# ChuyueL/advanced-hpc-lbm

Hardware: NVIDIA B200
Metric: MLUPS (d2q9-bgk lattice updates per second / 1e6) (higher is better)
Workload: dtype f32

## Files before the change

### advanced-hpc-lbm_b200/csrc/lbm_gpu.cu

```cuda
#include "lbm_gpu.h"
#include "lbm_kernels.cuh"
#include "lbm_cluster.cuh"
#include "lbm_tb2.cuh"
#include "lbm_tb3.cuh"
#include "lbm_pairs.cuh"
#include "lbm_f16.cuh"

#include <unistd.h>

#include <algorithm>
#include <cmath>
#include <cstdarg>
#include <cstdio>
#include <cstdlib>
#include <cstring>
#include <exception>
#include <memory>
#include <mutex>
#include <numeric>
#include <string>
#include <vector>

namespace {

thread_local std::string g_error;

struct CachedWindow { int device; size_t bytes; char* ptr; };
std::mutex g_window_mutex;
std::vector<CachedWindow> g_window_cache;
struct CachedIpcMapping { cudaIpcMemHandle_t handle; int device; void* ptr; };
std::vector<CachedIpcMapping> g_ipc_cache;

int fail(const char* fmt, ...) {
  char buf[1024];
  va_list ap;
  va_start(ap, fmt);
  vsnprintf(buf, sizeof buf, fmt, ap);
  va_end(ap);
  g_error = buf;
  return 1;
}

struct CudaError {
  std::string what;
};

#define CK(call)                                                                              \
  do {                                                                                        \
    cudaError_t e_ = (call);                                                                  \
    if (e_ != cudaSuccess) {                                                                  \
      char b_[512];                                                                           \
      snprintf(b_, sizeof b_, "CUDA error %s (%s) at %s:%d: %s", cudaGetErrorName(e_),        \
               cudaGetErrorString(e_), __FILE__, __LINE__, #call);                            \
      throw CudaError{b_};                                                                    \
    }                                                                                         \
  } while (0)

inline long long round_up(long long v, long long m) { return (v + m - 1) / m * m; }

inline bool env_on(const char* name) { const char* e = getenv(name); return e && e[0] == '1'; }

unsigned forced_kernel(unsigned flags) {
  static const char* const names[] = {nullptr, nullptr, "SCALAR", "TMA", "VEC4", nullptr, "PERSISTENT", nullptr, "CLUSTER", "TB2", nullptr, "PAIRS", "TB3"};
  unsigned k = 0;
  std::string msg = "more than one kernel forced, pass at most one of:";
  for (int b = 0; b < 13; b++)
    if (names[b] && (flags >> b & 1)) { k |= 1u << b; msg += std::string(" LBM_GPU_KERNEL_") + names[b]; }
  if (k & (k - 1)) throw CudaError{msg};
  return k;
}

constexpr int kPersistScalarBlocks = 296;
constexpr long long kPersistMaxCells = 1280 * 1024;
constexpr size_t kStagingBytes = 64u << 20;

struct IpcDesc {
  uint32_t magic;
  int32_t elem_size;
  int32_t device;
  int32_t pid;
  int32_t nx, pitch, rows;
  int32_t pad_;
  long long row0;
  unsigned long long win_addr;
  unsigned long long win_bytes;
  unsigned long long off_sync;
  unsigned long long off_gmask;
  unsigned long long steps_done;
  unsigned long long passes_done;
  long long local_free_cells;
  int32_t cur;
  int32_t tb2_ok;
  cudaIpcMemHandle_t handle;
  char gpu_uuid[16];
};
static_assert(sizeof(IpcDesc) <= LBM_GPU_IPC_DESC_BYTES, "descriptor too large");
constexpr uint32_t kIpcMagic = 0x4c424d31u;

enum SyncWord { kFlagFromBelow = 0, kFlagFromAbove = 1, kBoundaryDone = 2, kScratch0 = 3, kScratch1 = 4,
                kScratch2 = 5, kGridBarrier = 6, kAbort = 7, kSyncError = 8 ,
                kAvScratch = 16 , kSyncWords = 16 + 128 };
constexpr int kTb2MinRows = 8;
constexpr int kTb3MinRows = 12;
constexpr double kTb3MinWaves = 4.0;
constexpr int kAvWords = LBM_AV_STRIDE * LBM_AV_SLOTS;
constexpr int kMaxSegmentSteps = 1 << 16;

struct GridBase {
  virtual ~GridBase() {}
  virtual bool is_f64() const = 0;
};

template <typename real>
struct Slab {
  int device = 0;
  long long row0 = 0;
  int rows = 0;
  int accel_row = LBM_NO_ROW;
  char* base = nullptr;
  size_t bytes = 0;
  size_t off_lattice[2] = {0, 0}, off_side[2] = {0, 0}, off_mask = 0;
  real* lattice[2] = {nullptr, nullptr};
  real* side[2] = {nullptr, nullptr};
  uint32_t* mask = nullptr;
  char* win = nullptr;
  size_t win_bytes = 0, off_sync = 0, off_gmask = 0;
  unsigned long long* sync = nullptr;
  uint32_t* ghost_mask = nullptr;
  unsigned long long* av = nullptr;
  unsigned long long* av_compact = nullptr;
  size_t av_cap = 0;
  void* staging = nullptr;
  cudaStream_t stream = nullptr;
  cudaStream_t copy_stream = nullptr;
  cudaEvent_t stage_filled[2] = {nullptr, nullptr};
  cudaEvent_t stage_drained[2] = {nullptr, nullptr};
  cudaEvent_t ev0 = nullptr, ev1 = nullptr;
  cudaEvent_t step_ev[2] = {nullptr, nullptr};
  long long free_cells = 0;
  char* up_win = nullptr;
  char* dn_win = nullptr;
  unsigned long long* up_flag = nullptr;
  unsigned long long* dn_flag = nullptr;
  unsigned long long* up_abort = nullptr;
  unsigned long long* dn_abort = nullptr;
  uint32_t* up_gmask = nullptr;
  uint32_t* dn_gmask = nullptr;
  void* ipc_mapped[2] = {nullptr, nullptr};
  bool pooled = false;
  alignas(64) CUtensorMap tmap[2];
  alignas(64) CUtensorMap tmap_halo[2];
};

template <typename real> struct ParamT;
template <> struct ParamT<float> { typedef lbm_param type; };
template <> struct ParamT<double> { typedef lbm_param_f64 type; };

template <typename real>
class Grid : public GridBase {
 public:
  typedef typename ParamT<real>::type Param;
  Param prm;
  unsigned flags = 0;
  int kernel = 0;
  int persistent_vec = 4;
  int cluster_ctas = 0;
  int cluster_rows = 0;
  size_t cluster_smem = 0;
  int pitch = 0, mask_pitch = 0;
  bool slab_mode = false;
  bool connected = false;
  bool multi = false;
  bool use_flags = false;
  long long global_free_cells = -1;
  long long steps_done = 0;
  long long passes_done = 0;
  int cur = 0;
  int tb2_strips = 0, tb2_wout = 0, tb2_seg_rows = 0, tb2_span = 0, tb2_threads = 0;
  int tb2_tail_rows = 16, tb2_tail_segs = 0;
  int tb3_seg_rows = 0;
  int pairs_tile_rows = 0;
  bool f16 = false;
  bool failed = false;
  unsigned long long timeout_ns = 10000000000ULL;
  long long launches = 0;
  double last_run_ms = 0.0, last_step_ms = 0.0;
  std::vector<Slab<real>> slabs;

  bool is_f64() const override { return sizeof(real) == 8; }

  ~Grid() override {
    for (auto& s : slabs) {
      cudaSetDevice(s.device);
      if (s.stream) cudaStreamSynchronize(s.stream);
      for (int i = 0; i < 2; i++)
        if (s.ipc_mapped[i]) cudaIpcCloseMemHandle(s.ipc_mapped[i]);
      pool_free(s.av, s);
      pool_free(s.staging, s);
      pool_free(s.base, s);
      if (s.stream) cudaStreamSynchronize(s.stream);
      window_free(s);
      if (s.ev0) cudaEventDestroy(s.ev0);
      if (s.ev1) cudaEventDestroy(s.ev1);
      for (int i = 0; i < 2; i++) {
        if (s.stage_filled[i]) cudaEventDestroy(s.stage_filled[i]);
        if (s.stage_drained[i]) cudaEventDestroy(s.stage_drained[i]);
      }
      if (s.copy_stream) { cudaStreamSynchronize(s.copy_stream); cudaStreamDestroy(s.copy_stream); }
      for (int i = 0; i < 2; i++)
        if (s.step_ev[i]) cudaEventDestroy(s.step_ev[i]);
      if (s.stream) cudaStreamDestroy(s.stream);
    }
  }

  bool use_pool() const { return (flags & LBM_GPU_POOL) != 0; }
  void pool_alloc(void** p, size_t bytes, Slab<real>& s) {
    if (use_pool()) {
      int supported = 0;
      CK(cudaDeviceGetAttribute(&supported, cudaDevAttrMemoryPoolsSupported, s.device));
      if (supported) {
        cudaMemPool_t pool;
        CK(cudaDeviceGetDefaultMemPool(&pool, s.device));
        unsigned long long keep = ~0ULL;
        CK(cudaMemPoolSetAttribute(pool, cudaMemPoolAttrReleaseThreshold, &keep));
        CK(cudaMallocAsync(p, bytes, s.stream));
        s.pooled = true;
        return;
      }
    }
    CK(cudaMalloc(p, bytes));
  }
  static void pool_free(void* p, Slab<real>& s) {
    if (!p) return;
    if (s.pooled) cudaFreeAsync(p, s.stream);
    else cudaFree(p);
  }
  void window_alloc(Slab<real>& s) {
    if (use_pool()) {
      std::lock_guard<std::mutex> lock(g_window_mutex);
      for (size_t i = 0; i < g_window_cache.size(); i++)
        if (g_window_cache[i].device == s.device && g_window_cache[i].bytes == s.win_bytes) {
          s.win = g_window_cache[i].ptr;
          g_window_cache.erase(g_window_cache.begin() + i);
          return;
        }
    }
    CK(cudaMalloc((void**)&s.win, s.win_bytes));
  }
  void window_free(Slab<real>& s) {
    if (!s.win) return;
    if (use_pool()) {
      std::lock_guard<std::mutex> lock(g_window_mutex);
      g_window_cache.push_back({s.device, s.win_bytes, s.win});
    } else {
      cudaFree(s.win);
    }
    s.win = nullptr;
  }

  void alloc_slab(Slab<real>& s) {
    CK(cudaSetDevice(s.device));
    const long long plane = (long long)s.rows * pitch;
    const size_t lat = (size_t)9 * plane * (f16 ? sizeof(__half) : sizeof(real));
    const size_t side = (size_t)6 * pitch * sizeof(real);
    const size_t maskb = (size_t)s.rows * mask_pitch * sizeof(uint32_t);
    size_t off = 0;
    for (int i = 0; i < 2; i++) { s.off_lattice[i] = off; off = round_up(off + lat, 256); }
    for (int i = 0; i < 2; i++) { s.off_side[i] = off; off = round_up(off + side, 256); }
    s.off_mask = off; off = round_up(off + maskb, 256);
    s.bytes = off;
    CK(cudaStreamCreateWithFlags(&s.stream, cudaStreamNonBlocking));
    CK(cudaStreamCreateWithFlags(&s.copy_stream, cudaStreamNonBlocking));
    for (int i = 0; i < 2; i++) {
      CK(cudaEventCreateWithFlags(&s.stage_filled[i], cudaEventDisableTiming));
      CK(cudaEventCreateWithFlags(&s.stage_drained[i], cudaEventDisableTiming));
    }
    pool_alloc((void**)&s.base, s.bytes, s);
    for (int i = 0; i < 2; i++) {
      s.lattice[i] = (real*)(s.base + s.off_lattice[i]);
      s.side[i] = (real*)(s.base + s.off_side[i]);
    }
    s.mask = (uint32_t*)(s.base + s.off_mask);
    s.off_gmask = round_up((size_t)LBM_GHOST_PLANE_ROWS * pitch * sizeof(real), 256);
    s.off_sync = round_up(s.off_gmask + (size_t)2 * mask_pitch * sizeof(uint32_t), 256);
    s.win_bytes = round_up(s.off_sync + kSyncWords * sizeof(unsigned long long), 2u << 20);
    window_alloc(s);
    s.ghost_mask = (uint32_t*)(s.win + s.off_gmask);
    s.sync = (unsigned long long*)(s.win + s.off_sync);
    CK(cudaEventCreate(&s.ev0));
    CK(cudaEventCreate(&s.ev1));
    for (int i = 0; i < 2; i++) CK(cudaEventCreateWithFlags(&s.step_ev[i], cudaEventDisableTiming));
    CK(cudaMemsetAsync(s.base + s.off_side[0], 0, s.bytes - s.off_side[0], s.stream));
    CK(cudaMemsetAsync(s.win, 0, s.win_bytes, s.stream));
    void* st = nullptr;
    pool_alloc(&st, kStagingBytes, s);
    s.staging = st;
  }

  void make_tensor_maps(Slab<real>& s) {
    typedef CUresult (*EncodeFn)(CUtensorMap*, CUtensorMapDataType, cuuint32_t, void*, const cuuint64_t*,
                                 const cuuint64_t*, const cuuint32_t*, const cuuint32_t*, CUtensorMapInterleave,
                                 CUtensorMapSwizzle, CUtensorMapL2promotion, CUtensorMapFloatOOBfill);
    void* fn = nullptr;
    cudaDriverEntryPointQueryResult qres;
    CK(cudaGetDriverEntryPoint("cuTensorMapEncodeTiled", &fn, cudaEnableDefault, &qres));
    if (!fn || qres != cudaDriverEntryPointSuccess) throw CudaError{"cuTensorMapEncodeTiled is not available in this driver"};
    const cuuint64_t dims[3] = {(cuuint64_t)pitch, (cuuint64_t)s.rows, 9};
    const cuuint64_t strides[2] = {(cuuint64_t)pitch * sizeof(real), (cuuint64_t)plane_stride(s) * sizeof(real)};
    const cuuint32_t box[3] = {LBM_TMA_BOX, 1, 1};
    const cuuint32_t hbox[3] = {4, 1, 1};
    const cuuint32_t estr[3] = {1, 1, 1};
    for (int b = 0; b < 2; b++) {
      for (int h = 0; h < 2; h++) {
        const CUresult r = ((EncodeFn)fn)(h ? &s.tmap_halo[b] : &s.tmap[b], CU_TENSOR_MAP_DATA_TYPE_FLOAT32, 3, s.lattice[b],
                                          dims, strides, h ? hbox : box, estr, CU_TENSOR_MAP_INTERLEAVE_NONE,
                                          CU_TENSOR_MAP_SWIZZLE_NONE, CU_TENSOR_MAP_L2_PROMOTION_NONE,
                                          CU_TENSOR_MAP_FLOAT_OOB_FILL_NONE);
        if (r != CUDA_SUCCESS) {
          char msg[96];
          snprintf(msg, sizeof msg, "cuTensorMapEncodeTiled failed with CUresult %d", (int)r);
          throw CudaError{msg};
        }
      }
    }
  }

  real* win_section(char* win, int b, int d) const { return (real*)win + lbm::ghost_offset(pitch, b, d); }

  long long plane_stride(const Slab<real>& s) const { return (long long)s.rows * pitch; }

  __half* hlat(const Slab<real>& s, int b) const { return reinterpret_cast<__half*>(s.lattice[b]); }
  lbm::RestShift rest() const {
    lbm::RestShift r;
    r.w0 = (float)(prm.density * (real)4 / (real)9);
    r.w1 = (float)(prm.density / (real)9);
    r.w2 = (float)(prm.density / (real)36);
    return r;
  }

  void setup_geometry(int nx) {
    pitch = (int)round_up(nx, 32);
    mask_pitch = pitch / 32;
    if (const char* e = getenv("LBM_GPU_SYNC_TIMEOUT_MS")) {
      const double ms = atof(e);
      if (ms > 0) timeout_ns = (unsigned long long)(ms * 1e6);
    }
  }

  void tile_shape(int vec, int& bx, int& by) const {
    const int nxv = (prm.nx + vec - 1) / vec;
    bx = (int)std::min<long long>(LBM_BLOCK_THREADS, round_up(nxv, 32));
    if (kernel == LBM_GPU_KERNEL_TMA) bx = LBM_BLOCK_THREADS;
    by = LBM_BLOCK_THREADS / bx;
  }

  const void* persistent_fn() const {
    const bool strict = (flags & LBM_GPU_STRICT) != 0;
    if (persistent_vec == 1)
      return strict ? (const void*)lbm::lbm_steps_persistent<real, true, 1> : (const void*)lbm::lbm_steps_persistent<real, false, 1>;
    return strict ? (const void*)lbm::lbm_steps_persistent<real, true, 4> : (const void*)lbm::lbm_steps_persistent<real, false, 4>;
  }

  int persistent_capacity(const Slab<real>& s) {
    int per_sm = 0, sms = 0, coop = 0;
    CK(cudaOccupancyMaxActiveBlocksPerMultiprocessor(&per_sm, persistent_fn(), LBM_BLOCK_THREADS, 0));
    CK(cudaDeviceGetAttribute(&sms, cudaDevAttrMultiProcessorCount, s.device));
    CK(cudaDeviceGetAttribute(&coop, cudaDevAttrCooperativeLaunch, s.device));
    return coop ? per_sm * sms : 0;
  }

  const void* cluster_fn() const {
    return (flags & LBM_GPU_STRICT) ? (const void*)lbm::lbm_steps_cluster<true> : (const void*)lbm::lbm_steps_cluster<false>;
  }

  bool cluster_fits() {
    if (sizeof(real) != 4 || slabs.size() != 1 || slab_mode) return false;
    Slab<real>& s = slabs[0];
    int max_smem = 0;
    CK(cudaDeviceGetAttribute(&max_smem, cudaDevAttrMaxSharedMemoryPerBlockOptin, s.device));
    for (int c : {16, 8}) {
      const int rows = (s.rows + c - 1) / c;
      const size_t smem = (size_t)2 * 9 * rows * prm.nx * sizeof(float);
      if (smem > (size_t)max_smem) continue;
      if (cudaFuncSetAttribute(cluster_fn(), cudaFuncAttributeMaxDynamicSharedMemorySize, (int)smem) != cudaSuccess ||
          cudaFuncSetAttribute(cluster_fn(), cudaFuncAttributeNonPortableClusterSizeAllowed, 1) != cudaSuccess) {
        cudaGetLastError();
        continue;
      }
      cudaLaunchConfig_t cfg = {};
      cfg.gridDim = dim3(c);
      cfg.blockDim = dim3(LBM_CLUSTER_THREADS);
      cfg.dynamicSmemBytes = smem;
      cudaLaunchAttribute attr[1];
      attr[0].id = cudaLaunchAttributeClusterDimension;
      attr[0].val.clusterDim.x = c; attr[0].val.clusterDim.y = 1; attr[0].val.clusterDim.z = 1;
      cfg.attrs = attr;
      cfg.numAttrs = 1;
      int nclusters = 0;
      if (cudaOccupancyMaxActiveClusters(&nclusters, cluster_fn(), &cfg) != cudaSuccess || nclusters < 1) {
        cudaGetLastError();
        continue;
      }
      cluster_ctas = c;
      cluster_rows = rows;
      cluster_smem = smem;
      return true;
    }
// ... 1455 lines not shown
  return 0;
}

int lbm_gpu_ipc_export(lbm_gpu* h, void* desc) {
  if (!desc) return fail("lbm_gpu_ipc_export: NULL descriptor");
  return guarded<float>(h, "lbm_gpu_ipc_export", [&](Grid<float>& g) {
    if (g.slabs.size() != 1) throw CudaError{"only a one-slab handle can be exported"};
    if (g.f16) throw CudaError{"a LBM_GPU_STORE_F16 lattice cannot be shared between processes"};
    Slab<float>& s = g.slabs[0];
    CK(cudaSetDevice(s.device));
    IpcDesc d;
    memset(&d, 0, sizeof d);
    d.magic = kIpcMagic;
    d.elem_size = 4;
    d.device = s.device;
    d.pid = (int32_t)getpid();
    d.nx = g.prm.nx; d.pitch = g.pitch; d.rows = s.rows;
    d.row0 = s.row0;
    d.win_addr = (unsigned long long)(uintptr_t)s.win;
    d.win_bytes = s.win_bytes;
    d.off_sync = s.off_sync;
    d.off_gmask = s.off_gmask;
    d.steps_done = (unsigned long long)g.steps_done;
    d.passes_done = (unsigned long long)g.passes_done;
    d.local_free_cells = s.free_cells;
    d.cur = g.cur;
    d.tb2_ok = g.k7_fits(s.rows) ? 1 : 0;
    CK(cudaIpcGetMemHandle(&d.handle, s.win));
    cudaDeviceProp prop;
    CK(cudaGetDeviceProperties(&prop, s.device));
    memcpy(d.gpu_uuid, prop.uuid.bytes, 16);
    memset(desc, 0, LBM_GPU_IPC_DESC_BYTES);
    memcpy(desc, &d, sizeof d);
  });
}

namespace {
void ipc_connect_impl(Grid<float>& g, const IpcDesc& dn, const IpcDesc& up, bool ring_k7) {
  if (g.slabs.size() != 1) throw CudaError{"only a one-slab handle can be connected"};
  if (g.f16) throw CudaError{"a LBM_GPU_STORE_F16 lattice cannot be shared between processes"};
  Slab<float>& s = g.slabs[0];
  CK(cudaSetDevice(s.device));
  const long long ny = g.prm.ny;
  for (const IpcDesc* d : {&dn, &up}) {
    if (d->magic != kIpcMagic || d->elem_size != 4) throw CudaError{"bad neighbour descriptor"};
    if (d->nx != g.prm.nx || d->pitch != g.pitch) throw CudaError{"neighbour descriptor is for another grid width"};
    if (d->steps_done != (unsigned long long)g.steps_done || d->passes_done != (unsigned long long)g.passes_done ||
        d->cur != g.cur)
      throw CudaError{"neighbour is at a different timestep"};
  }
  cudaDeviceProp my_prop;
  CK(cudaGetDeviceProperties(&my_prop, s.device));
  for (const IpcDesc* d : {&dn, &up})
    if (memcmp(d->gpu_uuid, my_prop.uuid.bytes, 16) == 0 &&
        !(d->pid == (int32_t)getpid() && d->win_addr == (unsigned long long)(uintptr_t)s.win))
      throw CudaError{"a neighbouring slab runs on the same physical GPU: kernels that wait on one another "
                      "must not share a device (use lbm_gpu_create with n_gpus slabs in one process instead)"};
  if ((dn.row0 + dn.rows) % ny != s.row0 % ny) throw CudaError{"descriptor 'below' does not hold row0-1"};
  if ((s.row0 + s.rows) % ny != up.row0 % ny) throw CudaError{"descriptor 'above' does not hold row0+nrows"};
  auto map = [&](const IpcDesc& d, int slot) -> char* {
    if (d.pid == (int32_t)getpid()) {
      char* p = (char*)(uintptr_t)d.win_addr;
      if (p == s.win) return p;
      if (d.device == s.device)
        throw CudaError{"two slabs ordered by device-side flags must not share a GPU"};
      int can = 0;
      CK(cudaDeviceCanAccessPeer(&can, s.device, d.device));
      if (!can) throw CudaError{"peer access between the selected GPUs is not available"};
      cudaError_t e = cudaDeviceEnablePeerAccess(d.device, 0);
      if (e != cudaSuccess && e != cudaErrorPeerAccessAlreadyEnabled) CK(e);
      cudaGetLastError();
      return p;
    }
    if (g.use_pool()) {
      std::lock_guard<std::mutex> lock(g_window_mutex);
      for (auto& c : g_ipc_cache)
        if (c.device == s.device && memcmp(&c.handle, &d.handle, sizeof d.handle) == 0) return (char*)c.ptr;
    }
    void* p = nullptr;
    CK(cudaIpcOpenMemHandle(&p, d.handle, cudaIpcMemLazyEnablePeerAccess));
    if (g.use_pool()) {
      std::lock_guard<std::mutex> lock(g_window_mutex);
      g_ipc_cache.push_back({d.handle, s.device, p});
    } else {
      s.ipc_mapped[slot] = p;
    }
    return (char*)p;
  };
  for (const IpcDesc* d : {&dn, &up})
    if (d->win_bytes != s.win_bytes || d->off_sync != s.off_sync || d->off_gmask != s.off_gmask)
      throw CudaError{"neighbour window layout differs"};
  s.dn_win = map(dn, 0);
  s.up_win = (memcmp(&dn.handle, &up.handle, sizeof dn.handle) == 0 && dn.pid == up.pid) ? s.dn_win : map(up, 1);
  unsigned long long* dn_sync = (unsigned long long*)(s.dn_win + dn.off_sync);
  unsigned long long* up_sync = (unsigned long long*)(s.up_win + up.off_sync);
  s.dn_flag = dn_sync + kFlagFromAbove;
  s.up_flag = up_sync + kFlagFromBelow;
  s.dn_abort = dn_sync + kAbort;
  s.up_abort = up_sync + kAbort;
  s.dn_gmask = (uint32_t*)(s.dn_win + dn.off_gmask) + g.mask_pitch;
  s.up_gmask = (uint32_t*)(s.up_win + up.off_gmask);
  g.multi = true;
  g.use_flags = true;
  g.select_kernel(true, ring_k7);
  g.connected = true;
}
}

int lbm_gpu_ipc_connect(lbm_gpu* h, const void* desc_below, const void* desc_above) {
  if (!desc_below || !desc_above) return fail("lbm_gpu_ipc_connect: NULL descriptor");
  return guarded<float>(h, "lbm_gpu_ipc_connect", [&](Grid<float>& g) {
    IpcDesc dn, up;
    memcpy(&dn, desc_below, sizeof dn);
    memcpy(&up, desc_above, sizeof up);
    ipc_connect_impl(g, dn, up, false);
  });
}

int lbm_gpu_ipc_connect_all(lbm_gpu* h, const void* descs, int n) {
  if (!descs || n < 1) return fail("lbm_gpu_ipc_connect_all: bad argument");
  return guarded<float>(h, "lbm_gpu_ipc_connect_all", [&](Grid<float>& g) {
    if (g.slabs.size() != 1) throw CudaError{"only a one-slab handle can be connected"};
    Slab<float>& s = g.slabs[0];
    std::vector<IpcDesc> all(n);
    for (int i = 0; i < n; i++) memcpy(&all[i], (const char*)descs + (size_t)i * LBM_GPU_IPC_DESC_BYTES, sizeof(IpcDesc));
    const long long ny = g.prm.ny;
    long long rows_total = 0, free_total = 0;
    int below = -1, above = -1;
    bool all_k7 = true;
    for (int i = 0; i < n; i++) {
      const IpcDesc& d = all[i];
      if (d.magic != kIpcMagic) throw CudaError{"bad descriptor in the list"};
      rows_total += d.rows;
      free_total += d.local_free_cells;
      all_k7 = all_k7 && d.tb2_ok;
      if ((d.row0 + d.rows) % ny == s.row0 % ny) below = i;
      if ((s.row0 + s.rows) % ny == d.row0 % ny) above = i;
    }
    if (rows_total != ny) throw CudaError{"the descriptors do not cover the grid's rows exactly once"};
    if (below < 0 || above < 0) throw CudaError{"no descriptor holds the rows next to this slab"};
    ipc_connect_impl(g, all[below], all[above], all_k7);
    g.global_free_cells = free_total;
  });
}

int lbm_gpu_ipc_prepare(lbm_gpu* h) {
  return guarded<float>(h, "lbm_gpu_ipc_prepare", [&](Grid<float>& g) { g.prepare(); });
}

int lbm_gpu_run(lbm_gpu* h, int n_steps, float* av_vels_out) {
  return run_impl<float>(h, n_steps, av_vels_out, nullptr, "lbm_gpu_run");
}
int lbm_gpu_run_f64(lbm_gpu* h, int n_steps, double* av_vels_out) {
  return run_impl<double>(h, n_steps, av_vels_out, nullptr, "lbm_gpu_run_f64");
}
int lbm_gpu_run_batch(lbm_gpu* const* handles, int n, int n_steps, float* av_vels_out) {
  return run_batch_impl(handles, n, n_steps, av_vels_out);
}
int lbm_gpu_run_sums(lbm_gpu* h, int n_steps, double* sums_out) {
  if (!h) return fail("lbm_gpu_run_sums: NULL handle");
  if (reinterpret_cast<GridBase*>(h)->is_f64()) return run_impl<double>(h, n_steps, nullptr, sums_out, "lbm_gpu_run_sums");
  return run_impl<float>(h, n_steps, nullptr, sums_out, "lbm_gpu_run_sums");
}

int lbm_gpu_set_global_free_cells(lbm_gpu* h, long long free_cells) {
  if (!h) return fail("lbm_gpu_set_global_free_cells: NULL handle");
  if (free_cells < 1) return fail("lbm_gpu_set_global_free_cells: count must be positive");
  GridBase* b = reinterpret_cast<GridBase*>(h);
  if (b->is_f64()) static_cast<Grid<double>*>(b)->global_free_cells = free_cells;
  else static_cast<Grid<float>*>(b)->global_free_cells = free_cells;
  return 0;
}

int lbm_gpu_download(lbm_gpu* h, float* out) {
  if (!out) return fail("lbm_gpu_download: NULL output");
  return guarded<float>(h, "lbm_gpu_download", [&](Grid<float>& g) {
    long long rows = 0;
    for (auto& s : g.slabs) rows += s.rows;
    g.download_rows(g.slabs[0].row0, rows, out);
  });
}
int lbm_gpu_download_f64(lbm_gpu* h, double* out) {
  if (!out) return fail("lbm_gpu_download_f64: NULL output");
  return guarded<double>(h, "lbm_gpu_download_f64", [&](Grid<double>& g) {
    long long rows = 0;
    for (auto& s : g.slabs) rows += s.rows;
    g.download_rows(g.slabs[0].row0, rows, out);
  });
}
int lbm_gpu_download_rows(lbm_gpu* h, long long row0, long long nrows, float* out) {
  if (!out || nrows < 0) return fail("lbm_gpu_download_rows: bad argument");
  return guarded<float>(h, "lbm_gpu_download_rows", [&](Grid<float>& g) { g.download_rows(row0, nrows, out); });
}

int lbm_gpu_final_fields(lbm_gpu* h, long long row0, long long nrows, float* ux, float* uy, float* u, float* p) {
  if (nrows < 0) return fail("lbm_gpu_final_fields: bad argument");
  return guarded<float>(h, "lbm_gpu_final_fields", [&](Grid<float>& g) { g.final_fields(row0, nrows, ux, uy, u, p); });
}
int lbm_gpu_final_fields_f64(lbm_gpu* h, long long row0, long long nrows, double* ux, double* uy, double* u, double* p) {
  if (nrows < 0) return fail("lbm_gpu_final_fields_f64: bad argument");
  return guarded<double>(h, "lbm_gpu_final_fields_f64", [&](Grid<double>& g) { g.final_fields(row0, nrows, ux, uy, u, p); });
}

int lbm_gpu_coarse_fields(lbm_gpu* h, int factor, unsigned format, long long crow0, long long ncrows,
                          void* ux, void* uy, void* u, void* p) {
  if (factor < 1 || factor > 256) return fail("lbm_gpu_coarse_fields: factor %d is not in 1..256", factor);
  if (format != LBM_GPU_FIELDS_F32 && format != LBM_GPU_FIELDS_F16)
    return fail("lbm_gpu_coarse_fields: unknown format %u", format);
  if (ncrows < 0) return fail("lbm_gpu_coarse_fields: negative ncrows");
  if (h && reinterpret_cast<GridBase*>(h)->is_f64())
    return fail("lbm_gpu_coarse_fields: double-precision handles are not served (use lbm_gpu_final_fields_f64)");
  return guarded<float>(h, "lbm_gpu_coarse_fields", [&](Grid<float>& g) {
    void* const out[4] = {ux, uy, u, p};
    g.coarse_fields(factor, format == LBM_GPU_FIELDS_F16, crow0, ncrows, out);
  });
}

int lbm_gpu_av_velocity(lbm_gpu* h, float* av_out) {
  if (!av_out) return fail("lbm_gpu_av_velocity: NULL output");
  return guarded<float>(h, "lbm_gpu_av_velocity", [&](Grid<float>& g) {
    *av_out = (float)(g.av_velocity_sum() / (double)g.divisor());
  });
}
int lbm_gpu_av_velocity_f64(lbm_gpu* h, double* av_out) {
  if (!av_out) return fail("lbm_gpu_av_velocity_f64: NULL output");
  return guarded<double>(h, "lbm_gpu_av_velocity_f64", [&](Grid<double>& g) {
    *av_out = g.av_velocity_sum() / (double)g.divisor();
  });
}

int lbm_gpu_digest(lbm_gpu* h, double* total_density, unsigned long long* checksum) {
  if (!h) return fail("lbm_gpu_digest: NULL handle");
  if (reinterpret_cast<GridBase*>(h)->is_f64())
    return guarded<double>(h, "lbm_gpu_digest", [&](Grid<double>& g) { g.digest(total_density, checksum); });
  return guarded<float>(h, "lbm_gpu_digest", [&](Grid<float>& g) { g.digest(total_density, checksum); });
}

int lbm_gpu_upload(lbm_gpu* h, const float* cells_aos) {
  if (!cells_aos) return fail("lbm_gpu_upload: NULL input");
  return guarded<float>(h, "lbm_gpu_upload", [&](Grid<float>& g) {
    const int cur = g.cur;
    const long long base = g.slabs[0].row0;
    for (auto& s : g.slabs) g.upload_cells(s, cells_aos + (size_t)(s.row0 - base) * g.prm.nx * 9, cur);
    if (!g.slab_mode || g.slabs[0].rows == g.prm.ny) g.prepare();
  });
}
int lbm_gpu_upload_f64(lbm_gpu* h, const double* cells_aos) {
  if (!cells_aos) return fail("lbm_gpu_upload_f64: NULL input");
  return guarded<double>(h, "lbm_gpu_upload_f64", [&](Grid<double>& g) {
    const int cur = g.cur;
    for (auto& s : g.slabs) g.upload_cells(s, cells_aos + (size_t)s.row0 * g.prm.nx * 9, cur);
    g.prepare();
  });
}

int lbm_gpu_get_info(lbm_gpu* h, lbm_gpu_info* info) {
  if (!h || !info) return fail("lbm_gpu_get_info: NULL argument");
  memset(info, 0, sizeof *info);
  GridBase* b = reinterpret_cast<GridBase*>(h);
  auto fill = [&](auto& g) {
    info->nx = g.prm.nx; info->ny = g.prm.ny;
    info->n_gpus = (int)g.slabs.size();
    info->is_f64 = g.is_f64();
    info->kernel = g.kernel;
    info->pitch = g.pitch;
    info->local_free_cells = g.local_free_cells();
    info->free_cells = g.divisor();
    info->local_row0 = g.slabs[0].row0;
    long long rows = 0;
    size_t bytes = 0;
    for (auto& s : g.slabs) { rows += s.rows; bytes = std::max(bytes, s.bytes + kStagingBytes); }
    info->local_rows = rows;
    info->steps_done = g.steps_done;
    info->kernel_launches = g.launches;
    info->last_run_device_ms = g.last_run_ms;
    info->last_step_kernel_ms = g.last_step_ms;
    info->device_bytes = bytes;
  };
  if (b->is_f64()) fill(*static_cast<Grid<double>*>(b));
  else fill(*static_cast<Grid<float>*>(b));
  return 0;
}

int lbm_gpu_host_alloc(size_t bytes, void** out) {
  if (!out) return fail("lbm_gpu_host_alloc: NULL argument");
  *out = nullptr;
  cudaError_t e = cudaHostAlloc(out, bytes, cudaHostAllocPortable);
  if (e != cudaSuccess) {
    cudaGetLastError();
    return fail("lbm_gpu_host_alloc: %s", cudaGetErrorString(e));
  }
  return 0;
}

void lbm_gpu_host_free(void* p) {
  if (p) cudaFreeHost(p);
}

void lbm_gpu_destroy(lbm_gpu* h) {
  if (!h) return;
  delete reinterpret_cast<GridBase*>(h);
}

}
```

### advanced-hpc-lbm_b200/csrc/lbm_tb3.cuh

```cuda
#pragma once
#include "lbm_tb2.cuh"

namespace lbm {

#ifndef LBM_TB3_MIN_BLOCKS
#define LBM_TB3_MIN_BLOCKS (LBM_TB2_THREADS <= 64 ? 4 : LBM_TB2_THREADS <= 96 ? 3 : 2)
#endif

struct Tb3Level {
  float r13[2][2][LBM_TB2_ROWF];
  float r56[3][2][LBM_TB2_ROWF];
  float r78[2][LBM_TB2_ROWF];
};
struct Tb3Smem {
  float in[2][9][LBM_TB2_ROWF];
  Tb3Level lv[2];
  float p0[2][LBM_TB2_ROWF];
  unsigned long long mbar[2];
};
constexpr int kTb3PlaneRows = 18 + 2 * 12 + 2;
static_assert(sizeof(Tb3Smem) == kTb3PlaneRows * LBM_TB2_ROWF * sizeof(float) + 16, "ring layout");
static_assert((sizeof(Tb3Smem) + 512 + 1024) * LBM_TB3_MIN_BLOCKS <= 228 * 1024,
              "LBM_TB3_MIN_BLOCKS blocks of shared memory per SM");

__device__ __forceinline__ void tb3_init_smem(Tb3Smem& sm, const int span) {
  const int tid = threadIdx.x;
  for (int i = tid; i < kTb3PlaneRows * 2 * LBM_TB2_PAD; i += blockDim.x) {
    float* row = &sm.in[0][0][0] + (size_t)(i / (2 * LBM_TB2_PAD)) * LBM_TB2_ROWF;
    const int e = i % (2 * LBM_TB2_PAD);
    row[e < LBM_TB2_PAD ? e : span + e] = 0.f;
  }
  if (tid == 0) {
    asm volatile("mbarrier.init.shared::cta.b64 [%0], 1;" ::"r"(smem_u32(&sm.mbar[0])) : "memory");
    asm volatile("mbarrier.init.shared::cta.b64 [%0], 1;" ::"r"(smem_u32(&sm.mbar[1])) : "memory");
    asm volatile("fence.mbarrier_init.release.cluster;" ::: "memory");
  }
}

__device__ __forceinline__ void tb3_gather(const Tb3Level& L, const int c0, const int s13, const int s56,
                                           const float (&p0)[4], const float (&p2)[4], const float (&p4)[4],
                                           float (&in)[4][9]) {
#pragma unroll
  for (int j = 0; j < 4; j++) { in[j][0] = p0[j]; in[j][2] = p2[j]; in[j][4] = p4[j]; }
  tb2_get_west(L.r13[s13][0], c0, in[0][1], in[1][1], in[2][1], in[3][1]);
  tb2_get_east(L.r13[s13][1], c0, in[0][3], in[1][3], in[2][3], in[3][3]);
  tb2_get_west(L.r56[s56][0], c0, in[0][5], in[1][5], in[2][5], in[3][5]);
  tb2_get_east(L.r56[s56][1], c0, in[0][6], in[1][6], in[2][6], in[3][6]);
  tb2_get_east(L.r78[0], c0, in[0][7], in[1][7], in[2][7], in[3][7]);
  tb2_get_west(L.r78[1], c0, in[0][8], in[1][8], in[2][8], in[3][8]);
}
__device__ __forceinline__ void tb3_put_level(Tb3Level& L, const int c0, const int i, const float (&o)[4][9]) {
  tb2_put(L.r13[i & 1][0], c0, o, 1);
  tb2_put(L.r13[i & 1][1], c0, o, 3);
  tb2_put(L.r56[i % 3][0], c0, o, 5);
  tb2_put(L.r56[i % 3][1], c0, o, 6);
  tb2_put(L.r78[0], c0, o, 7);
  tb2_put(L.r78[1], c0, o, 8);
}

template <bool STRICT>
__device__ __forceinline__ void tb3_accelerate(const StepArgs<float>& a, float (&o)[4][9], const uint32_t mbits) {
#pragma unroll
  for (int j = 0; j < 4; j++)
    cell_accelerate<float, STRICT>(o[j][1], o[j][3], o[j][5], o[j][6], o[j][7], o[j][8], (mbits >> j) & 1u, a.aw1, a.aw2);
}

struct Tb3Carry {
  float p0[4];
  float p2a[4];
  float p2b[4];
  __device__ __forceinline__ void shift(const float (&o)[4][9]) {
#pragma unroll
    for (int j = 0; j < 4; j++) { p0[j] = o[j][0]; p2a[j] = p2b[j]; p2b[j] = o[j][2]; }
  }
};

template <bool STRICT>
__device__ __forceinline__ void tb3_tile(const Tb2Args& ta, Tb3Smem& sm, const int strip, const int seg,
                                         unsigned long long (&q)[3], bool (&bad)[3]) {
  const StepArgs<float>& a = ta.s;
  const int tid = threadIdx.x;
  const int X0 = strip * ta.wout;
  const int S0 = (X0 >= LBM_TB2_PAD) ? X0 - LBM_TB2_PAD : X0 - LBM_TB2_PAD + a.nx;
  const bool big = seg < ta.n_big;
  const int R0 = big ? seg * ta.seg_rows : ta.big_rows + (seg - ta.n_big) * ta.seg_rows_tail;
  const int R1 = big ? min(R0 + ta.seg_rows, ta.big_rows) : min(R0 + ta.seg_rows_tail, a.rows);
  const int n_it = R1 - R0 + 4;

  const int c0 = min(4 * tid, ta.span - 4);
  int xg = S0 + c0;
  while (xg >= a.nx) xg -= a.nx;
  const bool owned = (tid >= 1) && (4 * tid < ta.span) && (c0 - LBM_TB2_PAD < ta.wout) &&
                     (X0 + c0 - LBM_TB2_PAD < a.nx);

  const int my_plane = tb2_plane_of_thread();
  if (tid == 0) { tb2_expect(sm, 0, ta.span); tb2_expect(sm, 1, ta.span); }
#pragma unroll 1
  for (int k = 0; k < 2; k++) tb2_issue<true>(a, sm, k, R0 - 2 + k, S0, ta.span, my_plane);

  const QuadConsts<float, STRICT> qc(a.omega);
  const int mword_idx = xg >> 5, mshift = xg & 31;
  auto wrap = [&](const int row) { return (row < 0) ? row + a.rows : (row >= a.rows) ? row - a.rows : row; };
  auto mask_bits = [&](const int row) -> uint32_t {
    return (a.mask[(long long)wrap(row) * a.mask_pitch + mword_idx] >> mshift) & 0xFu;
  };
  uint32_t m1 = mask_bits(R0 - 2), m2 = 0u, m3 = 0u;
  Tb3Carry c1, c2;
  uint32_t phases = 0u;

#pragma unroll 1
  for (int i = 0; i < n_it; i++) {
    const int st = i & 1;
    const int r = R0 - 2 + i;
    const uint32_t m_next = (i + 1 < n_it) ? mask_bits(r + 1) : 0u;
    float in[4][9], out[4][9];
    bool b;
    tb2_mbar_wait(&sm.mbar[st], (phases >> st) & 1u);
    phases ^= 1u << st;
    if (tid == 0 && i + 2 < n_it) tb2_expect(sm, st, ta.span);
    {
      const float(*row)[LBM_TB2_ROWF] = sm.in[st];
      tb2_get(row[0], c0, in[0][0], in[1][0], in[2][0], in[3][0]);
      tb2_get(row[2], c0, in[0][2], in[1][2], in[2][2], in[3][2]);
      tb2_get(row[4], c0, in[0][4], in[1][4], in[2][4], in[3][4]);
      tb2_get_west(row[1], c0, in[0][1], in[1][1], in[2][1], in[3][1]);
      tb2_get_west(row[5], c0, in[0][5], in[1][5], in[2][5], in[3][5]);
      tb2_get_west(row[8], c0, in[0][8], in[1][8], in[2][8], in[3][8]);
      tb2_get_east(row[3], c0, in[0][3], in[1][3], in[2][3], in[3][3]);
      tb2_get_east(row[6], c0, in[0][6], in[1][6], in[2][6], in[3][6]);
      tb2_get_east(row[7], c0, in[0][7], in[1][7], in[2][7], in[3][7]);
    }
    unsigned long long qq = quad_update<float, STRICT>(in, m1, qc, out, b);
    if (owned && r >= R0 && r < R1) { q[0] += qq; bad[0] |= b; }
    if (wrap(r) == a.accel_row) tb3_accelerate<STRICT>(a, out, m1);
    tb3_put_level(sm.lv[0], c0, i, out);
    float p4[4];
#pragma unroll
    for (int j = 0; j < 4; j++) p4[j] = out[j][4];
    __syncthreads();
    if (i + 2 < n_it) tb2_issue<true>(a, sm, st, r + 2, S0, ta.span, my_plane);

    if (i >= 2) {
      const int y = r - 1;
      tb3_gather(sm.lv[0], c0, (i - 1) & 1, (i - 2) % 3, c1.p0, c1.p2a, p4, in);
      c1.shift(out);
      qq = quad_update<float, STRICT>(in, m2, qc, out, b);
      if (owned && y >= R0 && y < R1) { q[1] += qq; bad[1] |= b; }
      if (wrap(y) == a.accel_row) tb3_accelerate<STRICT>(a, out, m2);
      tb3_put_level(sm.lv[1], c0, i, out);
      tb2_put(sm.p0[i & 1], c0, out, 0);
      float n2[4];
#pragma unroll
      for (int j = 0; j < 4; j++) { n2[j] = out[j][2]; p4[j] = out[j][4]; }
      __syncthreads();

      if (i >= 4) {
        const int z = r - 2;
        tb3_gather(sm.lv[1], c0, (i - 1) & 1, (i - 2) % 3, c2.p2a, c2.p2a, p4, in);
        tb2_get(sm.p0[(i - 1) & 1], c0, in[0][0], in[1][0], in[2][0], in[3][0]);
        qq = quad_update<float, STRICT>(in, m3, qc, out, b);
        if (owned) {
          q[2] += qq;
          bad[2] |= b;
          tb2_store_row<STRICT>(a, z, xg, out, m3);
        }
      }
#pragma unroll
      for (int j = 0; j < 4; j++) { c2.p2a[j] = c2.p2b[j]; c2.p2b[j] = n2[j]; }
    } else {
      c1.shift(out);
    }
    m3 = m2;
    m2 = m1;
    m1 = m_next;
  }
}

template <bool STRICT>
__global__ void __launch_bounds__(LBM_TB2_THREADS, LBM_TB3_MIN_BLOCKS)
lbm_step3_tb(const __grid_constant__ Tb2Args ta) {
  extern __shared__ __align__(128) unsigned char tb3_smem_raw[];
  Tb3Smem& sm = *reinterpret_cast<Tb3Smem*>(tb3_smem_raw);
  const StepArgs<float>& a = ta.s;
  int strip, seg;
  tile_of_block(a.tiles_x, a.tiles_y, 1, strip, seg);
  tb3_init_smem(sm, ta.span);
  cudaGridDependencySynchronize();
  __syncthreads();
  unsigned long long q[3] = {0ULL, 0ULL, 0ULL};
  bool bad[3] = {false, false, false};
  tb3_tile<STRICT>(ta, sm, strip, seg, q, bad);
  if (bad[0]) atomicOr(a.av + 1, LBM_NONFINITE_MARK);
  if (bad[1]) atomicOr(ta.av2 + 1, LBM_NONFINITE_MARK);
  if (bad[2]) atomicOr(ta.av3 + 1, LBM_NONFINITE_MARK);
  block_accumulate(q[0], a.av);
  __syncthreads();
  block_accumulate(q[1], ta.av2);
  __syncthreads();
  block_accumulate(q[2], ta.av3);
}

}
```

Measured before the change: 175,500.

## Single-buffer TB3 input ring to fit more blocks per SM

Shrinks the three-step temporal-blocking kernel's input staging from two buffered rows with two mbarriers to a single buffer and one mbarrier, so the next row's load is issued only after the current row is consumed. The shared memory saved lets the minimum blocks per SM rise to four for up to 96 threads, and the wave threshold for choosing TB3 is lowered. It also adds optional cycle counters behind an experiments macro. The cost is less overlap between the bulk load and compute inside each block, which is traded for more resident blocks to hide that latency.

```diff
diff --git a/advanced-hpc-lbm_b200/csrc/lbm_gpu.cu b/advanced-hpc-lbm_b200/csrc/lbm_gpu.cu
--- a/advanced-hpc-lbm_b200/csrc/lbm_gpu.cu
+++ b/advanced-hpc-lbm_b200/csrc/lbm_gpu.cu
@@ -102,7 +102,7 @@
                 kAvScratch = 16 , kSyncWords = 16 + 128 };
 constexpr int kTb2MinRows = 8;
 constexpr int kTb3MinRows = 12;
-constexpr double kTb3MinWaves = 4.0;
+constexpr double kTb3MinWaves = 2.0;
 constexpr int kAvWords = LBM_AV_STRIDE * LBM_AV_SLOTS;
 constexpr int kMaxSegmentSteps = 1 << 16;
 
@@ -2164,4 +2164,15 @@
   delete reinterpret_cast<GridBase*>(h);
 }
 
-}
+#ifdef LBM_EXPERIMENTS
+int lbm_gpu_exp_tb3_cycles(unsigned long long out[2]) {
+  static const unsigned long long zero[2] = {0ULL, 0ULL};
+  if (cudaDeviceSynchronize() != cudaSuccess ||
+      cudaMemcpyFromSymbol(out, lbm::tb3_exp_cycles, sizeof zero) != cudaSuccess ||
+      cudaMemcpyToSymbol(lbm::tb3_exp_cycles, zero, sizeof zero) != cudaSuccess)
+    return fail("lbm_gpu_exp_tb3_cycles: %s", cudaGetErrorString(cudaGetLastError()));
+  return 0;
+}
+#endif
+
+}
diff --git a/advanced-hpc-lbm_b200/csrc/lbm_tb3.cuh b/advanced-hpc-lbm_b200/csrc/lbm_tb3.cuh
--- a/advanced-hpc-lbm_b200/csrc/lbm_tb3.cuh
+++ b/advanced-hpc-lbm_b200/csrc/lbm_tb3.cuh
@@ -4,7 +4,11 @@
 namespace lbm {
 
 #ifndef LBM_TB3_MIN_BLOCKS
-#define LBM_TB3_MIN_BLOCKS (LBM_TB2_THREADS <= 64 ? 4 : LBM_TB2_THREADS <= 96 ? 3 : 2)
+#define LBM_TB3_MIN_BLOCKS (LBM_TB2_THREADS <= 96 ? 4 : 2)
+#endif
+
+#ifdef LBM_EXPERIMENTS
+__device__ unsigned long long tb3_exp_cycles[2];
 #endif
 
 struct Tb3Level {
@@ -13,13 +17,13 @@
   float r78[2][LBM_TB2_ROWF];
 };
 struct Tb3Smem {
-  float in[2][9][LBM_TB2_ROWF];
+  float in[1][9][LBM_TB2_ROWF];
   Tb3Level lv[2];
   float p0[2][LBM_TB2_ROWF];
-  unsigned long long mbar[2];
+  unsigned long long mbar[1];
 };
-constexpr int kTb3PlaneRows = 18 + 2 * 12 + 2;
-static_assert(sizeof(Tb3Smem) == kTb3PlaneRows * LBM_TB2_ROWF * sizeof(float) + 16, "ring layout");
+constexpr int kTb3PlaneRows = 9 + 2 * 12 + 2;
+static_assert(sizeof(Tb3Smem) == kTb3PlaneRows * LBM_TB2_ROWF * sizeof(float) + 8, "ring layout");
 static_assert((sizeof(Tb3Smem) + 512 + 1024) * LBM_TB3_MIN_BLOCKS <= 228 * 1024,
               "LBM_TB3_MIN_BLOCKS blocks of shared memory per SM");
 
@@ -32,7 +36,6 @@
   }
   if (tid == 0) {
     asm volatile("mbarrier.init.shared::cta.b64 [%0], 1;" ::"r"(smem_u32(&sm.mbar[0])) : "memory");
-    asm volatile("mbarrier.init.shared::cta.b64 [%0], 1;" ::"r"(smem_u32(&sm.mbar[1])) : "memory");
     asm volatile("fence.mbarrier_init.release.cluster;" ::: "memory");
   }
 }
@@ -94,9 +97,8 @@
                      (X0 + c0 - LBM_TB2_PAD < a.nx);
 
   const int my_plane = tb2_plane_of_thread();
-  if (tid == 0) { tb2_expect(sm, 0, ta.span); tb2_expect(sm, 1, ta.span); }
-#pragma unroll 1
-  for (int k = 0; k < 2; k++) tb2_issue<true>(a, sm, k, R0 - 2 + k, S0, ta.span, my_plane);
+  if (tid == 0) tb2_expect(sm, 0, ta.span);
+  tb2_issue<true>(a, sm, 0, R0 - 2, S0, ta.span, my_plane);
 
   const QuadConsts<float, STRICT> qc(a.omega);
   const int mword_idx = xg >> 5, mshift = xg & 31;
@@ -106,20 +108,29 @@
   };
   uint32_t m1 = mask_bits(R0 - 2), m2 = 0u, m3 = 0u;
   Tb3Carry c1, c2;
-  uint32_t phases = 0u;
+  uint32_t phase = 0u;
+#ifdef LBM_EXPERIMENTS
+  const long long t_tile = clock64();
+  long long t_wait = 0;
+#endif
 
 #pragma unroll 1
   for (int i = 0; i < n_it; i++) {
-    const int st = i & 1;
     const int r = R0 - 2 + i;
     const uint32_t m_next = (i + 1 < n_it) ? mask_bits(r + 1) : 0u;
     float in[4][9], out[4][9];
     bool b;
-    tb2_mbar_wait(&sm.mbar[st], (phases >> st) & 1u);
-    phases ^= 1u << st;
-    if (tid == 0 && i + 2 < n_it) tb2_expect(sm, st, ta.span);
+#ifdef LBM_EXPERIMENTS
+    const long long t0 = clock64();
+    tb2_mbar_wait(&sm.mbar[0], phase);
+    t_wait += clock64() - t0;
+#else
+    tb2_mbar_wait(&sm.mbar[0], phase);
+#endif
+    phase ^= 1u;
+    if (tid == 0 && i + 1 < n_it) tb2_expect(sm, 0, ta.span);
     {
-      const float(*row)[LBM_TB2_ROWF] = sm.in[st];
+      const float(*row)[LBM_TB2_ROWF] = sm.in[0];
       tb2_get(row[0], c0, in[0][0], in[1][0], in[2][0], in[3][0]);
       tb2_get(row[2], c0, in[0][2], in[1][2], in[2][2], in[3][2]);
       tb2_get(row[4], c0, in[0][4], in[1][4], in[2][4], in[3][4]);
@@ -138,7 +149,7 @@
 #pragma unroll
     for (int j = 0; j < 4; j++) p4[j] = out[j][4];
     __syncthreads();
-    if (i + 2 < n_it) tb2_issue<true>(a, sm, st, r + 2, S0, ta.span, my_plane);
+    if (i + 1 < n_it) tb2_issue<true>(a, sm, 0, r + 1, S0, ta.span, my_plane);
 
     if (i >= 2) {
       const int y = r - 1;
@@ -174,6 +185,12 @@
     m2 = m1;
     m1 = m_next;
   }
+#ifdef LBM_EXPERIMENTS
+  if ((tid & 31) == 0) {
+    atomicAdd(&tb3_exp_cycles[0], (unsigned long long)t_wait);
+    atomicAdd(&tb3_exp_cycles[1], (unsigned long long)(clock64() - t_tile));
+  }
+#endif
 }
 
 template <bool STRICT>
```

Result: faster. 202,700, median of 6 (+15.5%).
